# JunweiLiang/FVTA_MemexQA

Measured on AMD Instinct MI355X. Metric: QA-pairs/sec (fwd+bwd) at B=64, 40 photos x 5 streams x 30 tok, h=512, higher is better.
Workload: dtype bf16; 1 GPU; BASELINE.json configs[2] train step (fwd+bwd+adam), shape 'metric', dense lengths; qa_pairs_per_gpu=64, albums=1, photos=40, text_streams=5, hidden=512, global_batch=64, K=6, T=1200, JQ=30, parallelism=dp1 (QA pairs sharded, flat-gradient all-reduce)

## Files before the change

### fvta_memexqa_amd/_lib.py

```python
import ctypes
import os
from ctypes import POINTER, Structure, c_char_p, c_float, c_int, c_int32, c_int64, c_size_t, c_void_p

_HERE = os.path.dirname(os.path.abspath(__file__))
LIB_PATH = os.environ.get("FVTA_LIB_PATH") or os.path.join(_HERE, "csrc", "libfvta_hip.so")

F32, BF16, BF16X3 = 0, 1, 2


class FvtaError(RuntimeError):
    pass


class AttnDesc(Structure):
    _fields_ = [(n, c_int32) for n in ("N", "K", "T", "JQ", "w", "simi", "feat_order", "add_tanh")] + [("hinfo_stride", c_int64)]


class LstmDesc(Structure):
    _fields_ = [(n, c_int32) for n in ("B", "J", "in_", "d", "share_fw_bw", "precision", "training", "reserved", "dx_overwrite", "out_pads_persist")] + \
               [("out_skip", c_int64)]


class TimewarpDesc(Structure):
    _fields_ = [(n, c_int32) for n in ("N", "K", "T", "w", "warp_type")] + [("window_t", c_float)]
# ... 18 lines not shown
class ContextDesc(Structure):
    _fields_ = [(n, c_int32) for n in ("N", "K", "M", "w")] + [("J", c_int32 * CTX_KMAX)]


class GuardDesc(Structure):
    _fields_ = [("grad_scale", c_float), ("clip_value", c_float), ("clip_norm", c_float), ("skip_nonfinite", c_int32),
                ("adam", c_int32), ("lr", c_float), ("beta1", c_float), ("beta2", c_float)]


class GuardCtl(Structure):
    _fields_ = [("grad_scale", c_float), ("clip_value", c_float), ("factor", c_float), ("lr_t", c_float), ("apply", c_int32),
                ("maxabs", c_float), ("norm", ctypes.c_double), ("nonfinite", c_int64), ("applied", c_int64),
                ("skipped", c_int64)]


P = c_void_p
_SIGS = {
    "fvta_version": (c_int, []),
    "fvta_last_error": (c_char_p, []),
    "fvta_abi_struct_bytes": (c_int64, [c_int32]),
    "fvta_attn_workspace_bytes": (c_size_t, [POINTER(AttnDesc)]),
    "fvta_attn_saved_bytes": (c_size_t, [POINTER(AttnDesc)]),
    "fvta_attn_plan": (c_int, [POINTER(AttnDesc), c_int32, POINTER(c_int32)]),
    "fvta_attn_fwd": (c_int, [POINTER(AttnDesc), P, P, P, P, P, P, P, P, P, P, P]),
    "fvta_attn_bwd": (c_int, [POINTER(AttnDesc), P, P, P, P, P, P, P, P, P, P, P, P, c_int, P, P]),
    "fvta_attn_fwd_shadow": (c_int, [POINTER(AttnDesc), P, P, P, P, P, P, P, P, P, P]),
    "fvta_attn_bwd_shadow": (c_int, [POINTER(AttnDesc), P, P, P, P, P, P, P, P, P, P, P, P, c_int, P, P]),
    "fvta_attn_fwd_tw": (c_int, [POINTER(AttnDesc), P, P, P, P, P, P, P, P, P, P, P, P]),
    "fvta_attn_bwd_tw": (c_int, [POINTER(AttnDesc), P, P, P, P, P, P, P, P, P, P, P, P, P, P, c_int, P, P]),
    "fvta_timewarp_bwd_att": (c_int, [POINTER(TimewarpDesc), P, P, P, P, P, P, P, P, P, P, P, P, P, P, P, P, P]),
    "fvta_lstm_plan_bytes": (c_size_t, [POINTER(LstmDesc)]),
    "fvta_lstm_saved_bytes": (c_size_t, [POINTER(LstmDesc)]),
    "fvta_lstm_workspace_bytes": (c_size_t, [POINTER(LstmDesc)]),
    "fvta_lstm_plan": (c_int, [POINTER(LstmDesc), P, P, P, P, c_int64, P, P]),
    "fvta_lstm_plan_xdir": (c_int, [POINTER(LstmDesc), P, P, P, P, c_int64, c_int64, P, P]),
    "fvta_dropout_pair_fwd": (c_int, [P, P, c_int64, c_float, ctypes.c_uint64, P]),
    "fvta_dropout_pair_bwd": (c_int, [P, P, c_int64, c_float, ctypes.c_uint64, c_int32, P]),
    "fvta_bilstm_fwd": (c_int, [POINTER(LstmDesc), P, P, P, P, P, P, P, P, P, P]),
    "fvta_bilstm_bwd": (c_int, [POINTER(LstmDesc), P, P, P, P, P, P, P, P, P, P, P, P, P, P]),
    "fvta_bilstm_bwd_overlap": (c_int, [POINTER(LstmDesc), P, P, P, P, P, P, P, P, P, P, P, P, P, P, P]),
    "fvta_bilstm_bwd_hint": (c_int, [POINTER(LstmDesc), P, P, P, P, P, P, P, P, P, P, P, P, P, P, P, P]),
    "fvta_lstm_shadow_rows": (c_int, [POINTER(LstmDesc), P, P, c_int64, P, P]),
    "fvta_rows_from_shadow": (c_int, [P, c_int64, c_int32, c_int64, P, P]),
    "fvta_lstm_last_state": (c_int, [POINTER(LstmDesc), P, P, c_int32, c_int32, P, P]),
    "fvta_lstm_last_state_bwd": (c_int, [POINTER(LstmDesc), P, P, c_int32, c_int32, P, P]),
    "fvta_scorer_ce_fwd": (c_int, [POINTER(ScorerDesc), P, P, P, P, P, P, P, P, P, P]),
    "fvta_scorer_ce_bwd": (c_int, [POINTER(ScorerDesc), P, P, P, P, P, P, P, P, c_float, P, P, P, P, P, P]),
    "fvta_attgru_fwd": (c_int, [c_int32, c_int32, P, P, P, P, P, P, P, P, P, P]),
    "fvta_attgru_bwd": (c_int, [c_int32, c_int32, P, P, P, P, P, P, P, P, P, P, P, P, P, P, P, P]),
    "fvta_timewarp_workspace_bytes": (c_size_t, [POINTER(TimewarpDesc)]),
    "fvta_timewarp_fwd": (c_int, [POINTER(TimewarpDesc), P, P, P, P, P, P, P, P, P, P, P]),
    "fvta_timewarp_bwd": (c_int, [POINTER(TimewarpDesc), P, P, P, P, P, P, P, P, P, P, P, P, P, P, P, P]),
    "fvta_timewarp_fwd_shadow": (c_int, [POINTER(TimewarpDesc), P, P, P, P, P, P, P, P, P, P, P]),
    "fvta_timewarp_bwd_shadow": (c_int, [POINTER(TimewarpDesc), P, P, P, P, P, P, P, P, P, P, P, P, P, P, P, P]),
    "fvta_embed_workspace_bytes": (c_size_t, [POINTER(EmbedDesc)]),
    "fvta_embed_fwd": (c_int, [POINTER(EmbedDesc), P, P, P, P, P, P, P, P, P, P, P]),
    "fvta_embed_bwd": (c_int, [POINTER(EmbedDesc), P, P, P, P, P, P, P, P, P, P, P, P, P]),
    "fvta_image_trans_fwd": (c_int, [POINTER(ImgTransDesc), P, P, P, P, P, P, P]),
    "fvta_image_trans_bwd": (c_int, [POINTER(ImgTransDesc), P, P, P, P, P, P, P, P, P]),
    "fvta_context_fwd": (c_int, [POINTER(ContextDesc), POINTER(P), POINTER(P), P, P, P]),
    "fvta_context_bwd": (c_int, [POINTER(ContextDesc), P, POINTER(P), P]),
    "fvta_adadelta_step": (c_int, [P, P, P, P, c_int64, c_float, c_float, c_float, c_float, P]),
    "fvta_adam_step": (c_int, [P, P, P, P, c_int64, c_float, c_float, c_float, c_float, c_int32, c_float, P]),
    "fvta_weight_decay": (c_int, [P, P, c_int64, c_float, P, P]),
    "fvta_grad_guard_workspace_bytes": (c_size_t, [c_int64]),
    "fvta_grad_guard": (c_int, [POINTER(GuardDesc), P, c_int64, P, P, P]),
# ... 86 lines not shown
```

### fvta_memexqa_amd/csrc/gemm_bf16.h

```cpp
#pragma once
#include "fvta_common.h"

namespace fvta {

typedef __attribute__((ext_vector_type(8))) __bf16 bf16x8_t;
typedef short s16x4 __attribute__((ext_vector_type(4)));
typedef __attribute__((address_space(3))) void* lds_void_ptr;

union Pack8 {
  bf16x8 s;
  bf16x8_t b;
  f32x4 f;
};

constexpr unsigned GLDS_OOB = 0x80000000u;

__device__ __forceinline__ __amdgpu_buffer_rsrc_t make_rsrc(const void* base, unsigned bytes) {
  return __builtin_amdgcn_make_buffer_rsrc(const_cast<void*>(base), 0, bytes, 0x00020000);
}
__device__ __forceinline__ void glds16(__amdgpu_buffer_rsrc_t rsrc, bf16_t* dst, unsigned voff, unsigned soff) {
  __builtin_amdgcn_raw_ptr_buffer_load_lds(rsrc, (lds_void_ptr)dst, 16, voff, soff, 0, 0);
}
template <int N>
__device__ __forceinline__ void wait_vmcnt() {
// ... 348 lines not shown
  FVTA_LS(2);
  for (int t = 0; t < ntiles; ++t) {
    const int ahead = min(S - 2, ntiles - 1 - t);
    if (ahead >= 3)
      wait_vmcnt<3 * G>();
    else if (ahead == 2)
      wait_vmcnt<2 * G>();
    else if (ahead == 1)
      wait_vmcnt<G>();
    else
      wait_vmcnt<0>();
    FVTA_LS(0);
    __builtin_amdgcn_s_barrier();
    asm volatile("" ::: "memory");
    FVTA_LS(1);
    if (t + S - 1 < ntiles) issue(t + S - 1, a_stage(t + S - 1), a_stage(t + S - 1) + TileCfg::A_ELEMS);
    FVTA_LS(2);
    const bf16_t* As = a_stage(t);
    if constexpr (KMAJOR)
      mma.compute_kmajor(As, As + TileCfg::A_ELEMS);
    else
      mma.compute_rows(As, As + TileCfg::A_ELEMS);
#ifdef FVTA_LOOP_STAMP
    asm volatile("s_nop 0" ::: "memory");
#endif
    FVTA_LS(3);
  }
#ifdef FVTA_LOOP_STAMP
  if (ls_on && mma.lane == 0)
    for (int i = 0; i < 4; ++i) g_loop_stamp[mma.wave_all][i] = ls_sum[i];
#endif
}

}
```

### fvta_memexqa_amd/csrc/lstm.hip

```cpp
#include "gemm_f32.h"
#include "fvta_prof.h"
#include <vector>

#include "lstm_common.h"

namespace fvta {

__device__ const float k_ones4[4] = {1.f, 0.f, 0.f, 0.f};


__global__ __launch_bounds__(1024) void plan_sort_kernel(PlanView v, const int32_t* __restrict__ len_in,
                                                         const int32_t* __restrict__ seq_J_in,
                                                         const int64_t* __restrict__ x_off_in,
                                                         const int64_t* __restrict__ out_off_in,
                                                         int64_t out_ld, int B, int J, int in, int d,
                                                         int64_t x_bw_delta) {
  extern __shared__ int32_t sh[];
  const int tid = threadIdx.x, wave = tid >> 6, lane = tid & 63;
  const int NW = 16, H = J + 1;
  for (int i = tid; i < NW * H; i += 1024) sh[i] = 0;
  const bool fresh = v.hdr->magic != PLAN_MAGIC || v.hdr->B != B || v.hdr->J != J || v.hdr->d != d || v.hdr->out_ld != out_ld;
  __syncthreads();
  if (tid == 0) {
    v.hdr->out_ld = out_ld;
// ... 471 lines not shown
    auto fb = [&](int k, int c, bool& ok) -> const float* { ok = k < K && n0 + c < N; return ok ? B + (size_t)k * N + n0 + c : B; };
    gemm_mainloop(mma, sa, sb, fa, fb, 0, Kp, smem, tid);
  }
#pragma unroll
  for (int ti = 0; ti < 2; ++ti)
#pragma unroll
    for (int r = 0; r < 16; ++r) {
      const int m = m0 + mma.row_of(ti, r);
#pragma unroll
      for (int tj = 0; tj < 2; ++tj) {
        const int n = n0 + mma.col_of(tj);
        if (m < M && n < N) C[(size_t)m * N + n] = mma.acc[ti][tj][r];
      }
    }
}

}

using namespace fvta;

static int check_lstm_desc(const fvta_lstm_desc* d) {
  FVTA_CHECK_ARG(d != nullptr, "lstm: null descriptor");
  FVTA_CHECK_ARG(d->B > 0 && d->J > 0 && d->J <= 1024, "lstm: need B>0 and 0<J<=1024 (B=%d J=%d)", d->B, d->J);
  FVTA_CHECK_ARG(d->in > 0 && d->in % 4 == 0, "lstm: input width must be a positive multiple of 4 (in=%d)", d->in);
  FVTA_CHECK_ARG(d->d > 0 && d->d % 32 == 0, "lstm: hidden size must be a positive multiple of 32 (d=%d)", d->d);
  FVTA_CHECK_ARG(d->precision == FVTA_F32 || d->precision == FVTA_BF16 || d->precision == FVTA_BF16X3,
                 "lstm: unknown precision %d", d->precision);
  return FVTA_OK;
}

extern "C" size_t fvta_lstm_plan_bytes(const fvta_lstm_desc* d) { return plan_view(d, nullptr).bytes; }
extern "C" size_t fvta_lstm_saved_bytes(const fvta_lstm_desc* d) { return saved_view(d, nullptr).bytes; }
extern "C" size_t fvta_lstm_workspace_bytes(const fvta_lstm_desc* d) { return work_view(d, nullptr).bytes; }

extern "C" int fvta_lstm_plan(const fvta_lstm_desc* d, const int32_t* len, const int32_t* seq_J,
                              const int64_t* x_off, const int64_t* out_off, int64_t out_ld, void* plan,
                              fvta_stream_t stream_) {
  return fvta_lstm_plan_xdir(d, len, seq_J, x_off, out_off, out_ld, 0, plan, stream_);
}

extern "C" int fvta_lstm_plan_xdir(const fvta_lstm_desc* d, const int32_t* len, const int32_t* seq_J,
                                   const int64_t* x_off, const int64_t* out_off, int64_t out_ld, int64_t x_bw_delta,
                                   void* plan, fvta_stream_t stream_) {
  if (int e = check_lstm_desc(d)) return e;
  FVTA_CHECK_ARG(len && seq_J && x_off && out_off && plan, "lstm_plan: null pointer");
  FVTA_CHECK_ARG(x_bw_delta >= 0 && x_bw_delta % 4 == 0, "lstm_plan: x_bw_delta=%lld must be >= 0 and a multiple of 4",
                 (long long)x_bw_delta);
  FVTA_CHECK_ARG(out_ld >= 2 * d->d && out_ld % 4 == 0, "lstm_plan: out_ld=%lld must be >= 2d and a multiple of 4",
                 (long long)out_ld);
  hipStream_t stream = (hipStream_t)stream_;
  PlanView v = plan_view(d, plan);
  const size_t sh = (size_t)16 * (d->J + 1) * sizeof(int32_t);
  hipLaunchKernelGGL(plan_sort_kernel, dim3(1), dim3(1024), sh, stream, v, len, seq_J, x_off, out_off, out_ld,
                     d->B, d->J, d->in, d->d, x_bw_delta);
  FVTA_CHECK_LAUNCH("plan_sort");
  hipLaunchKernelGGL(plan_fill_kernel, dim3((d->B + 255) / 256, d->J, 2), dim3(256), 0, stream, v, d->B, d->J,
                     d->in, d->d);
  FVTA_CHECK_LAUNCH("plan_fill");
  return FVTA_OK;
}

extern "C" int fvta_bilstm_fwd(const fvta_lstm_desc* d, const void* plan, const float* x, float* out,
                               const float* kernel_fw, const float* bias_fw, const float* kernel_bw,
                               const float* bias_bw, void* saved, void* workspace, fvta_stream_t stream_) {
  if (int e = check_lstm_desc(d)) return e;
  FVTA_CHECK_ARG(plan && x && out && kernel_fw && bias_fw && workspace, "bilstm_fwd: null pointer");
// ... 117 lines not shown
  s.W[1] = d->share_fw_bw ? kernel_fw : kernel_bw;
  s.dx = dx;
  s.dh_rec = wv.dh_rec;
  s.dzb = wv.dzb;
  s.in_i = in_internal(d);
  const int dbg = fvta_diag_env("FVTA_DEBUG_SKIP", 0);
  s.dbg = dbg;
  s.Wb[0] = wv.wb[0];
  s.Wb[1] = d->share_fw_bw ? wv.wb[0] : wv.wb[1];
  s.B = B;
  s.J = J;
  s.in = in;
  s.d = dd;
  const dim3 ggrid((unsigned)(((size_t)B * dd + 255) / 256), 1, 2);
  const dim3 sgrid((B + MmaSq::BM - 1) / MmaSq::BM, (in + dd + MmaSq::BN - 1) / MmaSq::BN, 2);
  const size_t sh = MmaSq::LDS_FLOATS * sizeof(float);
  DwArgs w;
  w.plan = pv;
  w.x = x;
  w.out = out;
  w.dz = sv.gates;
  w.slabs = wv.slabs;
  w.B = B;
  w.J = J;
  w.in = in;
  w.d = dd;
  w.tgroup = dw_tgroup(d);
  w.nsplit = dw_nsplit(d);
  w.dzb = wv.dzb;
  w.in_i = in_internal(d);
  w.xs = sv.xs;
  w.hs = sv.hs;
  w.xm = lstm_xm(d);
  (void)side_stream_;
  fvta_prof_begin(FVTA_PROF_LSTM_STEP_BWD + 16 * d->reserved, stream);
  if (bf) {
    FusedBwdArgs f;
    f.plan = pv;
    f.Wb[0] = wv.wb[0];
    f.Wb[1] = d->share_fw_bw ? wv.wb[0] : wv.wb[1];
    f.gatesb = sv.gatesb;
    f.cs = sv.cs;
    f.d_out = d_out;
    f.dzb = wv.dzb;
    f.dc = wv.cstate;
    f.dx = dx;
    f.B = B;
    f.J = J;
    f.in = in;
    f.d = dd;
    f.in_i = in_internal(d);
    f.gates32 = sv.gates;
    f.xm = lstm_xm(d);
    f.dx_accumulate = 1;
    f.dx_both = 0;
    if (dx && d->dx_overwrite) {
      const bool direct = dx_writes_whole_rows(f);
      hipLaunchKernelGGL(dx_zero_rows_kernel, dim3((B + 3) / 4), dim3(256), 0, stream, pv, dx, in, direct ? 1 : 0, B);
      f.dx_accumulate = direct ? 0 : 1;
    }
    for (int t = J - 1; t >= 0; --t) {
      f.t = t;
      f.nact_hint = nactive_host ? nactive_host[t] : -1;
      launch_bwd_fused_bf16(f, stream);
    }
    fvta_prof_end(FVTA_PROF_LSTM_STEP_BWD + 16 * d->reserved, J, stream);
    if (dx) {
      fvta_prof_begin(FVTA_PROF_LSTM_DX + 16 * d->reserved, stream);
      launch_dx_bf16(f, stream);
      fvta_prof_end(FVTA_PROF_LSTM_DX + 16 * d->reserved, 1, stream);
    }
  } else {
  if (dx && d->dx_overwrite) hipLaunchKernelGGL(dx_zero_rows_kernel, dim3((B + 3) / 4), dim3(256), 0, stream, pv, dx, in, 0, B);
  for (int t = J - 1; t >= 0; --t) {
    g.t = t;
    s.t = t;
    if (!(dbg & 512)) hipLaunchKernelGGL(lstm_gate_bwd, ggrid, dim3(256), 0, stream, g);
    if (t > 0 || dx) hipLaunchKernelGGL(lstm_step_bwd_f32, sgrid, dim3(256), sh, stream, s);
  }
  }
  if (!bf) fvta_prof_end(FVTA_PROF_LSTM_STEP_BWD + 16 * d->reserved, 2 * J, stream);
  FVTA_CHECK_LAUNCH("lstm_step_bwd");
  const int MM = in + dd + 1, N4 = 4 * dd;
  const dim3 wgrid((MM + MmaSq::BM - 1) / MmaSq::BM, N4 / MmaSq::BN, 2 * w.nsplit);
  fvta_prof_begin(FVTA_PROF_LSTM_DW + 16 * d->reserved, stream);
  if (dbg & 1024) {
  } else if (bf)
    launch_dw_bf16(w, stream);
  else
    hipLaunchKernelGGL(lstm_dw_f32, wgrid, dim3(256), sh, stream, w);
  FVTA_CHECK_LAUNCH("lstm_dw");
  const size_t slab_elems = bf ? (size_t)kpad8(d) * N4 : (size_t)MM * N4;
  const unsigned rgrid = (unsigned)((slab_elems + 255) / 256);
  if (bf) {
    const int ndir = d->share_fw_bw ? 1 : 2;
    for (int i = 0; i < ndir; ++i)
      launch_dw_reduce_bf16(wv.slabs + (size_t)i * w.nsplit * slab_elems, d->share_fw_bw ? 2 * w.nsplit : w.nsplit,
                            in, in_internal(d), dd, i == 0 ? dkernel_fw : dkernel_bw, i == 0 ? dbias_fw : dbias_bw,
                            stream);
  } else if (d->share_fw_bw) {
    hipLaunchKernelGGL(lstm_dw_reduce, dim3(rgrid), dim3(256), 0, stream, wv.slabs, 2 * w.nsplit, slab_elems,
                       in + dd, N4, dkernel_fw, dbias_fw);
  } else {
    hipLaunchKernelGGL(lstm_dw_reduce, dim3(rgrid), dim3(256), 0, stream, wv.slabs, w.nsplit, slab_elems, in + dd,
                       N4, dkernel_fw, dbias_fw);
    hipLaunchKernelGGL(lstm_dw_reduce, dim3(rgrid), dim3(256), 0, stream, wv.slabs + (size_t)w.nsplit * slab_elems,
                       w.nsplit, slab_elems, in + dd, N4, dkernel_bw, dbias_bw);
  }
  fvta_prof_end(FVTA_PROF_LSTM_DW + 16 * d->reserved, 1, stream);
  FVTA_CHECK_LAUNCH("lstm_dw_reduce");
  return FVTA_OK;
}

__global__ __launch_bounds__(256) void shadow_rows_kernel(PlanView v, const bf16_t* __restrict__ hs, int B, int J, int d,
                                                          int64_t nrows, unsigned long long* __restrict__ table) {
  const size_t idx = (size_t)blockIdx.x * blockDim.x + threadIdx.x;
  if (idx >= (size_t)2 * J * B) return;
  const int64_t oo = v.oo[idx];
  if (oo < 0) return;
  const int dir = (int)(idx / ((size_t)J * B));
  const int64_t row = oo / v.hdr->out_ld;
  if (row >= nrows) return;
  table[(size_t)dir * nrows + row] = (unsigned long long)reinterpret_cast<uintptr_t>(hs + idx * (size_t)d);
}
extern "C" int fvta_lstm_shadow_rows(const fvta_lstm_desc* d, const void* plan, const void* saved, int64_t nrows,
                                     uint64_t* table, fvta_stream_t stream) {
  if (int e = check_lstm_desc(d)) return e;
  FVTA_CHECK_ARG(plan && saved && table && nrows > 0, "lstm_shadow_rows: null pointer / no rows");
  FVTA_CHECK_ARG(d->precision == FVTA_BF16, "lstm_shadow_rows: the bf16 engine's shadow rows only");
  PlanView pv = plan_view(d, const_cast<void*>(plan));
// ... 79 lines not shown
```

### fvta_memexqa_amd/csrc/lstm_bf16.hip

```cpp
#include "gemm_bf16.h"
#include <type_traits>
#include "lstm_common.h"

namespace fvta {

static inline int pad8(int v) { return (v + 7) / 8 * 8; }

template <int B, int E, class F>
__device__ __forceinline__ void bf_static_for(F&& f) {
  if constexpr (B < E) {
    f(std::integral_constant<int, B>{});
    bf_static_for<B + 1, E>(f);
  }
}

template <class K>
static void allow_big_lds(K kernel, int bytes) {
  (void)hipFuncSetAttribute(reinterpret_cast<const void*>(kernel), hipFuncAttributeMaxDynamicSharedMemorySize, bytes);
}

__device__ __forceinline__ int il32(int e) { return ((e >> 5) << 6) + (e & 31); }
__global__ void cvt_weights_kernel(const float* __restrict__ W, bf16_t* __restrict__ wt, bf16_t* __restrict__ wb,
                                   int in, int in_i, int d, int xm) {
  __shared__ float tile[32][33];
// ... 557 lines not shown
    }
    for (int dir = 0; dir < 2; ++dir)
      hipLaunchKernelGGL((lstm_dx_bf16<2, FVTA_DX_BK, FVTA_DX_ST, false, false, XM>), grid, dim3(512), LDS, s, a, dir, a.dx_accumulate || dir);
    return;
  }
  constexpr int NBK = XM == 1 ? 32 : 64, NST = XM == 1 ? 3 : 2;
  if (XM == 2 && a.B <= 64 && a.in <= 128) {
    constexpr int LDSP = TileCfgT<4, 2, 1, NST, NBK, 1>::LDS_BYTES + 64 * 8;
    allow_big_lds(lstm_dx_bf16<4, NBK, NST, false, false, XM, 1, 1>, LDSP);
    const dim3 gridp((a.B + 63) / 64, 1, a.J);
    for (int dir = 0; dir < 2; ++dir)
      hipLaunchKernelGGL((lstm_dx_bf16<4, NBK, NST, false, false, XM, 1, 1>), gridp, dim3(256), LDSP, s, a, dir, a.dx_accumulate || dir);
    return;
  }
  constexpr int LDS1 = TileCfgT<1, 2, 4, NST, NBK>::LDS_BYTES + 256 * 8;
  allow_big_lds(lstm_dx_bf16<1, NBK, NST, false, false, XM>, LDS1);
  const dim3 grid(pad8((a.B + 255) / 256), (a.in + 127) / 128, a.J);
  for (int dir = 0; dir < 2; ++dir)
    hipLaunchKernelGGL((lstm_dx_bf16<1, NBK, NST, false, false, XM>), grid, dim3(256), LDS1, s, a, dir, a.dx_accumulate || dir);
}

void launch_dx_bf16(const FusedBwdArgs& a, hipStream_t s) {
  if (a.xm == 2)
    launch_dx_xm<2>(a, s);
  else
    launch_dx_xm<1>(a, s);
}

#ifndef FVTA_DW_STAGES
#define FVTA_DW_STAGES 4
#endif
constexpr int dw_stages(int wn) { return wn == 2 ? FVTA_DW_STAGES : 3; }

template <int WN>
__global__ __launch_bounds__((TileCfgT<WN>::NT), (WN == 1 ? 2 : 1)) void lstm_dw_bf16(DwArgs a) {
  typedef TileCfgT<WN, 2, 4, dw_stages(WN)> TileCfg;
  typedef MmaBT<WN, 2, 4, dw_stages(WN)> MmaB;
  extern __shared__ __attribute__((aligned(16))) bf16_t smem_h[];
  const int tid = threadIdx.x;
  const int d = a.d, in_i = a.in_i, N4 = 4 * d;
  const int xtiles = (in_i + TileCfg::BM - 1) / TileCfg::BM;
  const int mtiles = xtiles + (d + TileCfg::BM - 1) / TileCfg::BM, ntiles = N4 / TileCfg::BN, per = mtiles * ntiles;
  const int xcd = blockIdx.x & 7, slot = blockIdx.x >> 3;
  const int bz = xcd + 8 * (slot / per);
  const int tile_id = slot % per;
  if (bz >= 2 * a.nsplit) return;
  const int bx = tile_id % mtiles, by = tile_id / mtiles;
  const bool isx = bx < xtiles;
  const int col0 = isx ? bx * TileCfg::BM : (bx - xtiles) * TileCfg::BM;
  const int ncols = isx ? in_i : d;
  const int n0 = by * TileCfg::BN;
  const int split = bz % a.nsplit, dir = bz / a.nsplit;
  MmaB mma;
  mma.init(tid);
  KMajorSrc<TileCfg::BM, TileCfg::A_GLDS> sa;
  KMajorSrc<TileCfg::BN, TileCfg::B_GLDS> sb;
  sa.setup(mma.wave_all, mma.lane, col0, ncols, (unsigned)ncols * 2);
  sb.setup(mma.wave_all, mma.lane, n0, N4, (unsigned)N4 * 2);
  const int t_begin = split * a.tgroup, t_end = min(a.J, t_begin + a.tgroup);
  for (int t = t_begin; t < t_end; ++t) {
    const int nact = a.plan.nactive[t];
    if (nact == 0) break;
    if (!isx && t == 0) continue;
    const size_t trow = ((size_t)dir * a.J + t) * a.B;
    const bf16_t* A = isx ? a.xs + trow * in_i : a.hs + (trow - (size_t)a.B) * d;
    const __amdgpu_buffer_rsrc_t ra = make_rsrc(A, (unsigned)nact * ncols * 2);
    const __amdgpu_buffer_rsrc_t rz = make_rsrc(a.dzb + trow * (size_t)N4, (unsigned)nact * N4 * 2);
    auto issue = [&](int tile, bf16_t* As, bf16_t* Bs) {
      sa.issue(ra, As, mma.wave_all, (unsigned)tile * 32u * ncols * 2u);
      sb.issue(rz, Bs, mma.wave_all, (unsigned)tile * 32u * N4 * 2u);
    };
    glds_mainloop<true>(mma, issue, (nact + 31) / 32, smem_h);
    __builtin_amdgcn_s_barrier();
  }
  float* slab = a.slabs + (size_t)bz * (in_i + d) * N4;
  const int mrow0 = isx ? col0 : in_i + col0;
#pragma unroll
  for (int ti = 0; ti < MmaB::TM; ++ti)
#pragma unroll
    for (int r = 0; r < 16; ++r) {
      const int ml = mma.row_of(ti, r);
      if (col0 + ml >= ncols) continue;
#pragma unroll
      for (int tj = 0; tj < MmaB::TN; ++tj) slab[(size_t)(mrow0 + ml) * N4 + n0 + mma.col_of(tj)] = mma.acc[ti][tj][r];
    }
}

__global__ __launch_bounds__(512, 1) void lstm_dw_x2(DwArgs a) {
  typedef DwX2Cfg TileCfg;
  extern __shared__ __attribute__((aligned(16))) bf16_t smem_h[];
  const int tid = threadIdx.x;
  const int d = a.d, in_i = a.in_i, N4 = 4 * d;
  const int xtiles = (in_i + TileCfg::BM - 1) / TileCfg::BM;
  const int mtiles = xtiles + (d + TileCfg::BM - 1) / TileCfg::BM, ntiles = (N4 + TileCfg::BN - 1) / TileCfg::BN, per = mtiles * ntiles;
  const int xcd = blockIdx.x & 7, slot = blockIdx.x >> 3;
  const int bz = xcd + 8 * (slot / per);
  const int tile_id = slot % per;
  if (bz >= 2 * a.nsplit) return;
  const int bx = tile_id % mtiles, by = tile_id / mtiles;
  const bool isx = bx < xtiles;
  const int col0 = isx ? bx * TileCfg::BM : (bx - xtiles) * TileCfg::BM;
  const int ncols = isx ? in_i : d;
  const int n0 = by * TileCfg::BN;
  const int split = bz % a.nsplit, dir = bz / a.nsplit;
  MmaX2K mma;
  mma.init(tid);
  KMajorSrc<TileCfg::PCOLS, TileCfg::A_GLDS> sa;
  KMajorSrc<TileCfg::PCOLS, TileCfg::B_GLDS> sb;
  sa.setup(mma.wave_all, mma.lane, 2 * col0, 2 * ncols, (unsigned)ncols * 4);
  sb.setup(mma.wave_all, mma.lane, 2 * n0, 2 * N4, (unsigned)N4 * 4);
  const int t_begin = split * a.tgroup, t_end = min(a.J, t_begin + a.tgroup);
  for (int t = t_begin; t < t_end; ++t) {
    const int nact = a.plan.nactive[t];
    if (nact == 0) break;
    if (!isx && t == 0) continue;
    const size_t trow = ((size_t)dir * a.J + t) * a.B;
    const bf16_t* A = isx ? a.xs + trow * (size_t)(2 * in_i) : a.hs + (trow - (size_t)a.B) * (size_t)(2 * d);
    const __amdgpu_buffer_rsrc_t ra = make_rsrc(A, (unsigned)nact * ncols * 4);
    const __amdgpu_buffer_rsrc_t rz = make_rsrc(a.dzb + trow * (size_t)(2 * N4), (unsigned)nact * N4 * 4);
    auto issue = [&](int tile, bf16_t* As, bf16_t* Bs) {
      sa.issue(ra, As, mma.wave_all, (unsigned)tile * TileCfg::KR * ncols * 4u);
      sb.issue(rz, Bs, mma.wave_all, (unsigned)tile * TileCfg::KR * N4 * 4u);
    };
    glds_mainloop<true>(mma, issue, (nact + TileCfg::KR - 1) / TileCfg::KR, smem_h);
    __builtin_amdgcn_s_barrier();
  }
  float* slab = a.slabs + (size_t)bz * (in_i + d) * N4;
  const int mrow0 = isx ? col0 : in_i + col0;
#pragma unroll
  for (int ti = 0; ti < MmaX2K::TM; ++ti)
#pragma unroll
    for (int r = 0; r < 16; ++r) {
      const int ml = mma.row_of(ti, r);
      if (col0 + ml >= ncols) continue;
#pragma unroll
      for (int tj = 0; tj < MmaX2K::TN; ++tj)
        if (n0 + mma.col_of(tj) < N4) slab[(size_t)(mrow0 + ml) * N4 + n0 + mma.col_of(tj)] = mma.acc[ti][tj][r];
    }
}

void launch_dw_bf16(const DwArgs& a, hipStream_t s) {
  const int slices8 = (2 * a.nsplit + 7) / 8;
  if (a.xm == 2) {
    allow_big_lds(lstm_dw_x2, DwX2Cfg::LDS_BYTES);
    const int per = ((a.in_i + 255) / 256 + (a.d + 255) / 256) * ((4 * a.d + 255) / 256);
    hipLaunchKernelGGL(lstm_dw_x2, dim3(8 * per * slices8), dim3(512), DwX2Cfg::LDS_BYTES, s, a);
    return;
  }
  if ((4 * a.d) % 256 == 0) {
    constexpr int LDS2 = TileCfgT<2, 2, 4, dw_stages(2)>::LDS_BYTES;
    allow_big_lds(lstm_dw_bf16<2>, LDS2);
    const int per = ((a.in_i + 255) / 256 + (a.d + 255) / 256) * (4 * a.d / 256);
    hipLaunchKernelGGL((lstm_dw_bf16<2>), dim3(8 * per * slices8), dim3(512), LDS2, s, a);
  } else {
    allow_big_lds(lstm_dw_bf16<1>, TileCfgT<1>::LDS_BYTES);
    const int per = ((a.in_i + 255) / 256 + (a.d + 255) / 256) * (4 * a.d / 128);
    hipLaunchKernelGGL((lstm_dw_bf16<1>), dim3(8 * per * slices8), dim3(256), TileCfgT<1>::LDS_BYTES, s, a);
  }
}

__global__ __launch_bounds__(256) void lstm_dw_reduce_bf16(const float* __restrict__ slabs, int nslab, int in, int in_i, int d,
                                                            float* __restrict__ dW, float* __restrict__ dbias) {
  const int N4 = 4 * d;
  const size_t slab_elems = (size_t)(in_i + d) * N4;
  const size_t idx = ((size_t)blockIdx.x * blockDim.x + threadIdx.x) * 4;
  if (idx >= slab_elems) return;
  const int row = (int)(idx / N4), u = (int)(idx % N4) >> 2;
  if (row > in && row < in_i) return;
  f32x4 s = f32x4{0.f, 0.f, 0.f, 0.f};
  int k = 0;
  for (; k + 8 <= nslab; k += 8) {
    f32x4 v[8];
#pragma unroll
    for (int j = 0; j < 8; ++j) v[j] = *reinterpret_cast<const f32x4*>(slabs + (size_t)(k + j) * slab_elems + idx);
#pragma unroll
// ... 184 lines not shown
```

### fvta_memexqa_amd/csrc/lstm_common.h

```cpp
#pragma once
#include "fvta_common.h"

namespace fvta {

struct PlanHeader {
  int64_t out_ld;
  int32_t B, J, in, d;
  int64_t x_bw_delta;
  uint32_t magic;
  int32_t pad[7];
};
constexpr uint32_t PLAN_MAGIC = 0x46565441u;

struct PlanView {
  PlanHeader* hdr;
  int32_t* order;
  int32_t* nactive;
  int32_t* len;
  int32_t* seq_J;
  int64_t* x_off;
  int64_t* out_off;
  int64_t* xo;
  int64_t* oo;
  int32_t* dirty;
// ... 29 lines not shown
  bf16_t* gatesb;
  float* cs;
  bf16_t* xs;
  bf16_t* hs;
  size_t bytes;
};
static inline SavedView saved_view(const fvta_lstm_desc* d, void* p) {
  FvtaCarver c(p);
  SavedView s;
  s.gates = s.cs = nullptr;
  s.xs = s.hs = s.gatesb = nullptr;
  if (d->training) {
    if (d->precision == FVTA_BF16)
      s.gatesb = c.take<bf16_t>((size_t)2 * d->J * d->B * 4 * d->d);
    else
      s.gates = c.take<float>((size_t)2 * d->J * d->B * 4 * d->d);
    s.cs = c.take<float>((size_t)2 * d->J * d->B * d->d);
  }
  if (lstm_is_bf(d)) {
    s.xs = c.take<bf16_t>((size_t)2 * d->J * d->B * in_internal(d) * lstm_xm(d));
    s.hs = c.take<bf16_t>((size_t)2 * d->J * d->B * d->d * lstm_xm(d));
  }
  s.bytes = c.off < 256 ? 256 : c.off;
  return s;
}

static inline int dw_tgroup(const fvta_lstm_desc* d) {
  int g = (d->J + 15) / 16;
  return g < 1 ? 1 : g;
}
static inline int dw_nsplit(const fvta_lstm_desc* d) { return (d->J + dw_tgroup(d) - 1) / dw_tgroup(d); }
static inline int kpad8(const fvta_lstm_desc* d) { return in_internal(d) + d->d; }

struct WorkView {
  float* cstate;
  float* dh_rec;
  float* slabs;
  bf16_t* wt[2];
  bf16_t* wb[2];
  bf16_t* dzb;
  bf16_t* wf[2];
  size_t bytes;
};
static inline WorkView work_view(const fvta_lstm_desc* d, void* p) {
  FvtaCarver c(p);
  WorkView w;
  w.cstate = c.take<float>((size_t)2 * d->B * d->d);
  w.dh_rec = c.take<float>((size_t)2 * d->B * d->d);
  const size_t slab_rows = lstm_is_bf(d) ? (size_t)kpad8(d) : (size_t)(d->in + d->d + 1);
  w.slabs = c.take<float>((size_t)2 * dw_nsplit(d) * slab_rows * 4 * d->d);
  w.wt[0] = w.wt[1] = w.wb[0] = w.wb[1] = nullptr;
  w.dzb = nullptr;
  w.wf[0] = w.wf[1] = nullptr;
  if (lstm_is_bf(d)) {
    const size_t xm = (size_t)lstm_xm(d);
    for (int i = 0; i < 2; ++i) {
      w.wt[i] = c.take<bf16_t>((size_t)4 * d->d * kpad8(d) * xm);
      w.wb[i] = c.take<bf16_t>((size_t)kpad8(d) * 4 * d->d * xm);
    }
    if (d->training) w.dzb = c.take<bf16_t>((size_t)2 * d->J * d->B * 4 * d->d * xm);
    for (int i = 0; i < 2; ++i) w.wf[i] = c.take<bf16_t>((size_t)4 * d->d * kpad8(d) * xm);
  }
  w.bytes = c.off;
  return w;
}

struct StepArgs {
  PlanView plan;
  const float* x;
  float* out;
  const float* W[2];
  const bf16_t* Wt[2];
  const bf16_t* Wf[2];
  const bf16_t* xs;
  bf16_t* hs;
  const float* bias[2];
  float* gates;
  bf16_t* gatesb;
  float* cs;
  float* cstate;
  int t, B, J, in, d, Kp;
  int dbg;
  int xm;
  int nt;
  int64_t out_skip;
};

struct GateBwdArgs {
  PlanView plan;
  const float* d_out;
  float* gates;
  const bf16_t* gatesb;
  bf16_t* dzb;
  const float* cs;
  float* dc;
  float* dh_rec;
  int t, B, J, d;
};

struct StepBwdArgs {
  PlanView plan;
  const float* dz;
  const bf16_t* dzb;
  const float* W[2];
  const bf16_t* Wb[2];
  float* dx;
  float* dh_rec;
  int t, B, J, in, d, in_i;
  int dbg;
};

struct DwArgs {
  PlanView plan;
  const float* x;
  const float* out;
  const float* dz;
  const bf16_t* dzb;
  const bf16_t* xs;
  const bf16_t* hs;
  float* slabs;
  int B, J, in, d, tgroup, nsplit, in_i;
  int xm;
};

#ifdef __HIPCC__
template <class Mma>
__device__ __forceinline__ void lstm_gate_epilogue(const Mma& mma, const StepArgs& a, int dir, int m0, int u0,
                                                   int nact, size_t trow, const int64_t* s_oo) {
  static_assert(Mma::TN == 4 && Mma::WAVES_N == 1, "wave tile must span the four gate strips");
  const int d = a.d, t = a.t;
  const float* __restrict__ bias = a.bias[dir];
  const int u = u0 + mma.l31;
  const float bi = bias[u], bj = bias[d + u], bf = bias[2 * d + u], bo = bias[3 * d + u];
  const float* cprev_src = a.cs ? a.cs + (trow - a.B) * (size_t)d : a.cstate + (size_t)dir * a.B * d;
#pragma unroll
  for (int ti = 0; ti < Mma::TM; ++ti) {
    float cp[16];
#pragma unroll
    for (int r = 0; r < 16; ++r) {
      const int i = min(m0 + mma.row_of(ti, r), nact - 1);
      cp[r] = (t > 0 && !(a.dbg & 64)) ? cprev_src[(size_t)i * d + u] : 0.f;
    }
#pragma unroll
    for (int r = 0; r < 16; ++r) {
      const int row = mma.row_of(ti, r);
      const int i = m0 + row;
      const float ig = fvta_sigmoid(mma.acc[ti][0][r] + bi);
      const float jg = fvta_tanh(mma.acc[ti][1][r] + bj);
      const float fg = fvta_sigmoid(mma.acc[ti][2][r] + bf + 1.0f);
      const float og = fvta_sigmoid(mma.acc[ti][3][r] + bo);
      const float c = cp[r] * fg + ig * jg;
      const float h = fvta_tanh(c) * og;
      if (i < nact) {
        if (a.cs) {
          if (!(a.dbg & 16)) a.cs[(trow + i) * d + u] = c;
// ... 194 lines not shown
```

### include/fvta_hip.h

```cpp
#ifndef FVTA_HIP_H
#define FVTA_HIP_H

#include <stddef.h>
#include <stdint.h>

#ifdef __cplusplus
extern "C" {
#endif

#define FVTA_OK 0
#define FVTA_ERR_INVALID_ARG (-1)
#define FVTA_ERR_LAUNCH (-2)
#define FVTA_ERR_UNSUPPORTED (-3)

#define FVTA_F32 0
#define FVTA_BF16 1
#define FVTA_BF16X3 2

typedef void* fvta_stream_t;

int fvta_version(void);
const char* fvta_last_error(void);
int64_t fvta_abi_struct_bytes(int32_t which);

// ... 21 lines not shown
int fvta_attn_fwd_shadow(const fvta_attn_desc* d, const uint64_t* table, const float* hq, const uint8_t* hmask,
                         const uint8_t* qmask, const float* W, const float* b, float* h_a, void* saved, void* workspace,
                         fvta_stream_t stream);
int fvta_attn_bwd_shadow(const fvta_attn_desc* d, const uint64_t* table, const float* hq, const uint8_t* hmask,
                         const uint8_t* qmask, const float* W, const float* b, const float* d_h_a, const void* saved,
                         float* d_hinfo, float* d_hq, float* dW, float* db, int accumulate, void* workspace,
                         fvta_stream_t stream);

int fvta_attn_fwd_tw(const fvta_attn_desc* d, const float* hinfo, const float* hq, const uint8_t* hmask,
                     const uint8_t* qmask, const float* W, const float* b, const float* tscale, float* h_a,
                     float* a_logits, void* saved, void* workspace, fvta_stream_t stream);
int fvta_attn_bwd_tw(const fvta_attn_desc* d, const float* hinfo, const float* hq, const uint8_t* hmask,
                     const uint8_t* qmask, const float* W, const float* b, const float* tscale, const float* d_h_a,
                     const void* saved, float* d_hinfo, float* d_hq, float* dW, float* db, float* d_tscale,
                     int accumulate, void* workspace, fvta_stream_t stream);

typedef struct fvta_lstm_desc {
  int32_t B;
  int32_t J;
  int32_t in;
  int32_t d;
  int32_t share_fw_bw;
  int32_t precision;
  int32_t training;
  int32_t reserved;
  int32_t dx_overwrite;
  int32_t out_pads_persist;
  int64_t out_skip;
} fvta_lstm_desc;

size_t fvta_lstm_plan_bytes(const fvta_lstm_desc* d);
size_t fvta_lstm_saved_bytes(const fvta_lstm_desc* d);
size_t fvta_lstm_workspace_bytes(const fvta_lstm_desc* d);

int fvta_lstm_plan(const fvta_lstm_desc* d, const int32_t* len, const int32_t* seq_J, const int64_t* x_off,
                   const int64_t* out_off, int64_t out_ld, void* plan, fvta_stream_t stream);

int fvta_lstm_plan_xdir(const fvta_lstm_desc* d, const int32_t* len, const int32_t* seq_J, const int64_t* x_off,
                        const int64_t* out_off, int64_t out_ld, int64_t x_bw_delta, void* plan, fvta_stream_t stream);
int fvta_dropout_pair_fwd(const float* x, float* x2, int64_t n, float keep_prob, uint64_t seed, fvta_stream_t stream);
int fvta_dropout_pair_bwd(const float* dx2, float* dx, int64_t n, float keep_prob, uint64_t seed, int32_t accumulate,
                          fvta_stream_t stream);

int fvta_bilstm_fwd(const fvta_lstm_desc* d, const void* plan, const float* x, float* out,
                    const float* kernel_fw, const float* bias_fw, const float* kernel_bw,
                    const float* bias_bw, void* saved, void* workspace, fvta_stream_t stream);

int fvta_bilstm_bwd(const fvta_lstm_desc* d, const void* plan, const float* x, const float* out,
                    const float* d_out, const float* kernel_fw, const float* kernel_bw, void* saved,
                    float* dx, float* dkernel_fw, float* dbias_fw, float* dkernel_bw, float* dbias_bw,
                    void* workspace, fvta_stream_t stream);

int fvta_bilstm_bwd_overlap(const fvta_lstm_desc* d, const void* plan, const float* x, const float* out,
                            const float* d_out, const float* kernel_fw, const float* kernel_bw, void* saved,
                            float* dx, float* dkernel_fw, float* dbias_fw, float* dkernel_bw, float* dbias_bw,
                            void* workspace, fvta_stream_t stream, fvta_stream_t side_stream);

int fvta_bilstm_bwd_hint(const fvta_lstm_desc* d, const void* plan, const float* x, const float* out,
                         const float* d_out, const float* kernel_fw, const float* kernel_bw, void* saved,
                         float* dx, float* dkernel_fw, float* dbias_fw, float* dkernel_bw, float* dbias_bw,
                         void* workspace, fvta_stream_t stream, fvta_stream_t side_stream, const int32_t* nactive_host);

int fvta_lstm_shadow_rows(const fvta_lstm_desc* d, const void* plan, const void* saved, int64_t nrows, uint64_t* table,
                          fvta_stream_t stream);
int fvta_rows_from_shadow(const uint64_t* table, int64_t nrows, int32_t d, int64_t out_ld, float* out, fvta_stream_t stream);
int fvta_lstm_last_state(const fvta_lstm_desc* d, const void* plan, const float* out, int32_t s0,
// ... 202 lines not shown
```

Measured before the change: 5402 QA-pairs/s.

## Balance LSTM weight-gradient work by k-tile slices across timesteps

```diff
diff --git a/fvta_memexqa_amd/_lib.py b/fvta_memexqa_amd/_lib.py
--- a/fvta_memexqa_amd/_lib.py
+++ b/fvta_memexqa_amd/_lib.py
@@ -74,6 +74,8 @@
     "fvta_lstm_plan_bytes": (c_size_t, [POINTER(LstmDesc)]),
     "fvta_lstm_saved_bytes": (c_size_t, [POINTER(LstmDesc)]),
     "fvta_lstm_workspace_bytes": (c_size_t, [POINTER(LstmDesc)]),
+    "fvta_lstm_dw_nslices": (c_int, [POINTER(LstmDesc)]),
+    "fvta_lstm_dw_slices": (c_int, [POINTER(c_int32), c_int32, c_int32, c_int32, c_int32, POINTER(c_int32)]),
     "fvta_lstm_plan": (c_int, [POINTER(LstmDesc), P, P, P, P, c_int64, P, P]),
     "fvta_lstm_plan_xdir": (c_int, [POINTER(LstmDesc), P, P, P, P, c_int64, c_int64, P, P]),
     "fvta_dropout_pair_fwd": (c_int, [P, P, c_int64, c_float, ctypes.c_uint64, P]),
diff --git a/fvta_memexqa_amd/csrc/gemm_bf16.h b/fvta_memexqa_amd/csrc/gemm_bf16.h
--- a/fvta_memexqa_amd/csrc/gemm_bf16.h
+++ b/fvta_memexqa_amd/csrc/gemm_bf16.h
@@ -404,4 +404,38 @@
 #endif
 }
 
-}
+template <class Mma, class Cursor>
+__device__ __forceinline__ void glds_mainloop_kmajor_steps(Mma& mma, Cursor& cur, int ntiles, bf16_t* smem) {
+  typedef typename Mma::Cfg TileCfg;
+  constexpr int S = TileCfg::STAGES, G = TileCfg::A_GLDS + TileCfg::B_GLDS;
+  static_assert(S >= 3 && S <= 5, "ring depth");
+  if (ntiles <= 0) return;
+#pragma unroll
+  for (int p = 0; p < S - 1; ++p) {
+    bf16_t* st = smem + p * TileCfg::STAGE_ELEMS;
+    cur.issue(st, st + TileCfg::A_ELEMS);
+    cur.advance();
+    cur.prefetch();
+    cur.settle();
+  }
+  cur.prefetch();
+  int is = S - 1, cs = 0;
+  for (int i = 0; i < ntiles; ++i) {
+    wait_vmcnt<(S - 2) * G>();
+    __builtin_amdgcn_s_barrier();
+    asm volatile("" ::: "memory");
+    cur.settle();
+    bf16_t* st = smem + is * TileCfg::STAGE_ELEMS;
+    cur.issue(st, st + TileCfg::A_ELEMS);
+    cur.advance();
+    const bf16_t* As = smem + cs * TileCfg::STAGE_ELEMS;
+    mma.compute_kmajor(As, As + TileCfg::A_ELEMS);
+    cur.prefetch();
+    is = is + 1 == S ? 0 : is + 1;
+    cs = cs + 1 == S ? 0 : cs + 1;
+  }
+  cur.settle();
+  wait_vmcnt<0>();
+}
+
+}
diff --git a/fvta_memexqa_amd/csrc/lstm.hip b/fvta_memexqa_amd/csrc/lstm.hip
--- a/fvta_memexqa_amd/csrc/lstm.hip
+++ b/fvta_memexqa_amd/csrc/lstm.hip
@@ -527,6 +527,30 @@
 extern "C" size_t fvta_lstm_plan_bytes(const fvta_lstm_desc* d) { return plan_view(d, nullptr).bytes; }
 extern "C" size_t fvta_lstm_saved_bytes(const fvta_lstm_desc* d) { return saved_view(d, nullptr).bytes; }
 extern "C" size_t fvta_lstm_workspace_bytes(const fvta_lstm_desc* d) { return work_view(d, nullptr).bytes; }
+
+extern "C" int fvta_lstm_dw_nslices(const fvta_lstm_desc* d) {
+  if (check_lstm_desc(d)) return -1;
+  return lstm_is_bf(d) ? dw_nslices(d) : 0;
+}
+extern "C" int fvta_lstm_dw_slices(const int32_t* nactive, int32_t J, int32_t KR, int32_t NS, int32_t htile, int32_t* out) {
+  FVTA_CHECK_ARG(nactive && out, "lstm_dw_slices: null pointer");
+  FVTA_CHECK_ARG(J > 0 && KR > 0 && NS > 0, "lstm_dw_slices: need J, KR, NS > 0 (J=%d KR=%d NS=%d)", J, KR, NS);
+  for (int t = 0; t < J; ++t)
+    FVTA_CHECK_ARG(nactive[t] >= 0 && (t == 0 || nactive[t] <= nactive[t - 1]),
+                   "lstm_dw_slices: nactive must be non-negative and non-increasing (step %d)", t);
+  for (int s = 0; s < NS; ++s) {
+    const DwSlice sl = dw_slice_range(nactive, J, KR, NS, s, htile != 0);
+    int32_t* o = out + 5 * s;
+    o[0] = o[1] = o[2] = o[3] = -1;
+    o[4] = sl.n;
+    if (sl.n <= 0) continue;
+    int t = sl.t, k = sl.k;
+    for (int i = 1; i < sl.n; ++i)
+      if (++k >= dw_ktiles(nactive[t], KR)) ++t, k = 0;
+    o[0] = sl.t, o[1] = sl.k, o[2] = t, o[3] = k;
+  }
+  return FVTA_OK;
+}
 
 extern "C" int fvta_lstm_plan(const fvta_lstm_desc* d, const int32_t* len, const int32_t* seq_J,
                               const int64_t* x_off, const int64_t* out_off, int64_t out_ld, void* plan,
@@ -710,6 +734,7 @@
   w.xs = sv.xs;
   w.hs = sv.hs;
   w.xm = lstm_xm(d);
+  w.nslices = bf ? dw_nslices(d) : 0;
   (void)side_stream_;
   fvta_prof_begin(FVTA_PROF_LSTM_STEP_BWD + 16 * d->reserved, stream);
   if (bf) {
@@ -773,7 +798,7 @@
   if (bf) {
     const int ndir = d->share_fw_bw ? 1 : 2;
     for (int i = 0; i < ndir; ++i)
-      launch_dw_reduce_bf16(wv.slabs + (size_t)i * w.nsplit * slab_elems, d->share_fw_bw ? 2 * w.nsplit : w.nsplit,
+      launch_dw_reduce_bf16(wv.slabs + (size_t)i * w.nslices * slab_elems, d->share_fw_bw ? 2 * w.nslices : w.nslices,
                             in, in_internal(d), dd, i == 0 ? dkernel_fw : dkernel_bw, i == 0 ? dbias_fw : dbias_bw,
                             stream);
   } else if (d->share_fw_bw) {
diff --git a/fvta_memexqa_amd/csrc/lstm_bf16.hip b/fvta_memexqa_amd/csrc/lstm_bf16.hip
--- a/fvta_memexqa_amd/csrc/lstm_bf16.hip
+++ b/fvta_memexqa_amd/csrc/lstm_bf16.hip
@@ -613,6 +613,71 @@
 #endif
 constexpr int dw_stages(int wn) { return wn == 2 ? FVTA_DW_STAGES : 3; }
 
+
+struct DwPlace {
+  int bz;
+  int dir, slice, col0, ncols, n0;
+  bool isx;
+};
+template <int BM, int BN>
+__device__ __forceinline__ DwPlace dw_place(const DwArgs& a) {
+  const int N4 = 4 * a.d;
+  const int xtiles = (a.in_i + BM - 1) / BM;
+  const int mtiles = xtiles + (a.d + BM - 1) / BM, ntiles = (N4 + BN - 1) / BN, per = mtiles * ntiles;
+  const int xcd = blockIdx.x & 7, slot = blockIdx.x >> 3;
+  const int tile_id = slot % per, bx = tile_id % mtiles, by = tile_id / mtiles;
+  DwPlace p;
+  p.bz = xcd + 8 * (slot / per);
+  p.isx = bx < xtiles;
+  p.col0 = p.isx ? bx * BM : (bx - xtiles) * BM;
+  p.ncols = p.isx ? a.in_i : a.d;
+  p.n0 = by * BN;
+  p.slice = p.bz % a.nslices, p.dir = p.bz / a.nslices;
+  return p;
+}
+
+typedef const __attribute__((address_space(4))) int32_t* dw_nact_ptr;
+template <int KR, class SA, class SB>
+struct DwCursor {
+  const SA& sa;
+  const SB& sb;
+  dw_nact_ptr nactive;
+  const bf16_t *abase, *zbase;
+  int a_back;
+  size_t a_step, z_step;
+  unsigned a_ld, z_ld;
+  int J, wave;
+  int t, k, nk, nact, nact_nx, left;
+  __device__ __forceinline__ DwCursor(const SA& sa_, const SB& sb_) : sa(sa_), sb(sb_) {}
+  __device__ __forceinline__ void start(const DwSlice& sl) {
+    t = sl.t, k = sl.k, left = sl.n;
+    nact = nactive[min(t, J)];
+    nk = dw_ktiles(nact, KR);
+    prefetch();
+    settle();
+  }
+  __device__ __forceinline__ void issue(bf16_t* As, bf16_t* Bs) const {
+    const unsigned rows = left > 0 ? (unsigned)nact : 0u;
+    const __amdgpu_buffer_rsrc_t ra = make_rsrc(abase + (size_t)(t - a_back) * a_step, rows * a_ld);
+    const __amdgpu_buffer_rsrc_t rz = make_rsrc(zbase + (size_t)t * z_step, rows * z_ld);
+    sa.issue(ra, As, wave, (unsigned)k * KR * a_ld);
+    sb.issue(rz, Bs, wave, (unsigned)k * KR * z_ld);
+  }
+  __device__ __forceinline__ void advance() {
+    const bool wrap = k + 1 >= nk;
+    left -= 1;
+    k = wrap ? 0 : k + 1;
+    t = wrap ? t + 1 : t;
+    nact = wrap ? nact_nx : nact;
+    nk = dw_ktiles(nact, KR);
+  }
+  __device__ __forceinline__ void prefetch() {
+    dw_nact_ptr p = nactive + min(t + 1, J);
+    asm volatile("s_load_dword %0, %1, 0x0" : "=s"(nact_nx) : "s"(p) : "memory");
+  }
+  __device__ __forceinline__ void settle() { asm volatile("s_waitcnt lgkmcnt(0)" : "+s"(nact_nx)::"memory"); }
+};
+
 template <int WN>
 __global__ __launch_bounds__((TileCfgT<WN>::NT), (WN == 1 ? 2 : 1)) void lstm_dw_bf16(DwArgs a) {
   typedef TileCfgT<WN, 2, 4, dw_stages(WN)> TileCfg;
@@ -620,41 +685,31 @@
   extern __shared__ __attribute__((aligned(16))) bf16_t smem_h[];
   const int tid = threadIdx.x;
   const int d = a.d, in_i = a.in_i, N4 = 4 * d;
-  const int xtiles = (in_i + TileCfg::BM - 1) / TileCfg::BM;
-  const int mtiles = xtiles + (d + TileCfg::BM - 1) / TileCfg::BM, ntiles = N4 / TileCfg::BN, per = mtiles * ntiles;
-  const int xcd = blockIdx.x & 7, slot = blockIdx.x >> 3;
-  const int bz = xcd + 8 * (slot / per);
-  const int tile_id = slot % per;
-  if (bz >= 2 * a.nsplit) return;
-  const int bx = tile_id % mtiles, by = tile_id / mtiles;
-  const bool isx = bx < xtiles;
-  const int col0 = isx ? bx * TileCfg::BM : (bx - xtiles) * TileCfg::BM;
-  const int ncols = isx ? in_i : d;
-  const int n0 = by * TileCfg::BN;
-  const int split = bz % a.nsplit, dir = bz / a.nsplit;
+  const DwPlace p = dw_place<TileCfg::BM, TileCfg::BN>(a);
+  if (p.bz >= 2 * a.nslices) return;
+  const bool isx = p.isx;
+  const int col0 = p.col0, ncols = p.ncols, n0 = p.n0;
   MmaB mma;
   mma.init(tid);
-  KMajorSrc<TileCfg::BM, TileCfg::A_GLDS> sa;
-  KMajorSrc<TileCfg::BN, TileCfg::B_GLDS> sb;
+  typedef KMajorSrc<TileCfg::BM, TileCfg::A_GLDS> SrcA;
+  typedef KMajorSrc<TileCfg::BN, TileCfg::B_GLDS> SrcB;
+  SrcA sa;
+  SrcB sb;
   sa.setup(mma.wave_all, mma.lane, col0, ncols, (unsigned)ncols * 2);
   sb.setup(mma.wave_all, mma.lane, n0, N4, (unsigned)N4 * 2);
-  const int t_begin = split * a.tgroup, t_end = min(a.J, t_begin + a.tgroup);
-  for (int t = t_begin; t < t_end; ++t) {
-    const int nact = a.plan.nactive[t];
-    if (nact == 0) break;
-    if (!isx && t == 0) continue;
-    const size_t trow = ((size_t)dir * a.J + t) * a.B;
-    const bf16_t* A = isx ? a.xs + trow * in_i : a.hs + (trow - (size_t)a.B) * d;
-    const __amdgpu_buffer_rsrc_t ra = make_rsrc(A, (unsigned)nact * ncols * 2);
-    const __amdgpu_buffer_rsrc_t rz = make_rsrc(a.dzb + trow * (size_t)N4, (unsigned)nact * N4 * 2);
-    auto issue = [&](int tile, bf16_t* As, bf16_t* Bs) {
-      sa.issue(ra, As, mma.wave_all, (unsigned)tile * 32u * ncols * 2u);
-      sb.issue(rz, Bs, mma.wave_all, (unsigned)tile * 32u * N4 * 2u);
-    };
-    glds_mainloop<true>(mma, issue, (nact + 31) / 32, smem_h);
-    __builtin_amdgcn_s_barrier();
-  }
-  float* slab = a.slabs + (size_t)bz * (in_i + d) * N4;
+  DwCursor<32, SrcA, SrcB> cur(sa, sb);
+  cur.nactive = (dw_nact_ptr)a.plan.nactive;
+  cur.J = a.J, cur.wave = mma.wave_all;
+  const size_t row0 = (size_t)p.dir * a.J * a.B;
+  cur.abase = isx ? a.xs + row0 * in_i : a.hs + row0 * d;
+  cur.a_back = isx ? 0 : 1;
+  cur.zbase = a.dzb + row0 * (size_t)N4;
+  cur.a_step = (size_t)a.B * ncols, cur.z_step = (size_t)a.B * N4;
+  cur.a_ld = (unsigned)ncols * 2, cur.z_ld = (unsigned)N4 * 2;
+  const DwSlice sl = dw_slice_range(cur.nactive, a.J, 32, a.nslices, p.slice, !isx);
+  cur.start(sl);
+  glds_mainloop_kmajor_steps(mma, cur, sl.n, smem_h);
+  float* slab = a.slabs + (size_t)p.bz * (in_i + d) * N4;
   const int mrow0 = isx ? col0 : in_i + col0;
 #pragma unroll
   for (int ti = 0; ti < MmaB::TM; ++ti)
@@ -672,41 +727,31 @@
   extern __shared__ __attribute__((aligned(16))) bf16_t smem_h[];
   const int tid = threadIdx.x;
   const int d = a.d, in_i = a.in_i, N4 = 4 * d;
-  const int xtiles = (in_i + TileCfg::BM - 1) / TileCfg::BM;
-  const int mtiles = xtiles + (d + TileCfg::BM - 1) / TileCfg::BM, ntiles = (N4 + TileCfg::BN - 1) / TileCfg::BN, per = mtiles * ntiles;
-  const int xcd = blockIdx.x & 7, slot = blockIdx.x >> 3;
-  const int bz = xcd + 8 * (slot / per);
-  const int tile_id = slot % per;
-  if (bz >= 2 * a.nsplit) return;
-  const int bx = tile_id % mtiles, by = tile_id / mtiles;
-  const bool isx = bx < xtiles;
-  const int col0 = isx ? bx * TileCfg::BM : (bx - xtiles) * TileCfg::BM;
-  const int ncols = isx ? in_i : d;
-  const int n0 = by * TileCfg::BN;
-  const int split = bz % a.nsplit, dir = bz / a.nsplit;
+  const DwPlace p = dw_place<TileCfg::BM, TileCfg::BN>(a);
+  if (p.bz >= 2 * a.nslices) return;
+  const bool isx = p.isx;
+  const int col0 = p.col0, ncols = p.ncols, n0 = p.n0;
   MmaX2K mma;
   mma.init(tid);
-  KMajorSrc<TileCfg::PCOLS, TileCfg::A_GLDS> sa;
-  KMajorSrc<TileCfg::PCOLS, TileCfg::B_GLDS> sb;
+  typedef KMajorSrc<TileCfg::PCOLS, TileCfg::A_GLDS> SrcA;
+  typedef KMajorSrc<TileCfg::PCOLS, TileCfg::B_GLDS> SrcB;
+  SrcA sa;
+  SrcB sb;
   sa.setup(mma.wave_all, mma.lane, 2 * col0, 2 * ncols, (unsigned)ncols * 4);
   sb.setup(mma.wave_all, mma.lane, 2 * n0, 2 * N4, (unsigned)N4 * 4);
-  const int t_begin = split * a.tgroup, t_end = min(a.J, t_begin + a.tgroup);
-  for (int t = t_begin; t < t_end; ++t) {
-    const int nact = a.plan.nactive[t];
-    if (nact == 0) break;
-    if (!isx && t == 0) continue;
-    const size_t trow = ((size_t)dir * a.J + t) * a.B;
-    const bf16_t* A = isx ? a.xs + trow * (size_t)(2 * in_i) : a.hs + (trow - (size_t)a.B) * (size_t)(2 * d);
-    const __amdgpu_buffer_rsrc_t ra = make_rsrc(A, (unsigned)nact * ncols * 4);
-    const __amdgpu_buffer_rsrc_t rz = make_rsrc(a.dzb + trow * (size_t)(2 * N4), (unsigned)nact * N4 * 4);
-    auto issue = [&](int tile, bf16_t* As, bf16_t* Bs) {
-      sa.issue(ra, As, mma.wave_all, (unsigned)tile * TileCfg::KR * ncols * 4u);
-      sb.issue(rz, Bs, mma.wave_all, (unsigned)tile * TileCfg::KR * N4 * 4u);
-    };
-    glds_mainloop<true>(mma, issue, (nact + TileCfg::KR - 1) / TileCfg::KR, smem_h);
-    __builtin_amdgcn_s_barrier();
-  }
-  float* slab = a.slabs + (size_t)bz * (in_i + d) * N4;
+  DwCursor<TileCfg::KR, SrcA, SrcB> cur(sa, sb);
+  cur.nactive = (dw_nact_ptr)a.plan.nactive;
+  cur.J = a.J, cur.wave = mma.wave_all;
+  const size_t row0 = (size_t)p.dir * a.J * a.B;
+  cur.abase = isx ? a.xs + row0 * (size_t)(2 * in_i) : a.hs + row0 * (size_t)(2 * d);
+  cur.a_back = isx ? 0 : 1;
+  cur.zbase = a.dzb + row0 * (size_t)(2 * N4);
+  cur.a_step = (size_t)a.B * 2 * ncols, cur.z_step = (size_t)a.B * 2 * N4;
+  cur.a_ld = (unsigned)ncols * 4, cur.z_ld = (unsigned)N4 * 4;
+  const DwSlice sl = dw_slice_range(cur.nactive, a.J, TileCfg::KR, a.nslices, p.slice, !isx);
+  cur.start(sl);
+  glds_mainloop_kmajor_steps(mma, cur, sl.n, smem_h);
+  float* slab = a.slabs + (size_t)p.bz * (in_i + d) * N4;
   const int mrow0 = isx ? col0 : in_i + col0;
 #pragma unroll
   for (int ti = 0; ti < MmaX2K::TM; ++ti)
@@ -721,7 +766,7 @@
 }
 
 void launch_dw_bf16(const DwArgs& a, hipStream_t s) {
-  const int slices8 = (2 * a.nsplit + 7) / 8;
+  const int slices8 = (2 * a.nslices + 7) / 8;
   if (a.xm == 2) {
     allow_big_lds(lstm_dw_x2, DwX2Cfg::LDS_BYTES);
     const int per = ((a.in_i + 255) / 256 + (a.d + 255) / 256) * ((4 * a.d + 255) / 256);
diff --git a/fvta_memexqa_amd/csrc/lstm_common.h b/fvta_memexqa_amd/csrc/lstm_common.h
--- a/fvta_memexqa_amd/csrc/lstm_common.h
+++ b/fvta_memexqa_amd/csrc/lstm_common.h
@@ -85,6 +85,64 @@
 static inline int dw_nsplit(const fvta_lstm_desc* d) { return (d->J + dw_tgroup(d) - 1) / dw_tgroup(d); }
 static inline int kpad8(const fvta_lstm_desc* d) { return in_internal(d) + d->d; }
 
+#if defined(__HIPCC__)
+#define FVTA_HD __host__ __device__
+#else
+#define FVTA_HD
+#endif
+struct DwSlice {
+  int t, k;
+  int n;
+};
+FVTA_HD inline int dw_ktiles(int nact, int KR) { return nact > 0 ? (nact + KR - 1) / KR : 0; }
+template <class NactPtr>
+FVTA_HD inline DwSlice dw_slice_range(NactPtr nactive, int J, int KR, int NS, int s, bool htile) {
+  const int tb = htile ? 1 : 0;
+  long long T = 0;
+  for (int t0 = tb; t0 < J; t0 += 8) {
+    int nk[8];
+#pragma unroll
+    for (int u = 0; u < 8; ++u) nk[u] = dw_ktiles(nactive[t0 + u < J ? t0 + u : J - 1], KR);
+#pragma unroll
+    for (int u = 0; u < 8; ++u) T += t0 + u < J ? nk[u] : 0;
+  }
+  const long long lo = s * T / NS, hi = (s + 1) * T / NS;
+  DwSlice r;
+  r.t = tb;
+  r.k = 0;
+  r.n = (int)(hi - lo);
+  long long before = 0;
+  bool found = false;
+  for (int t0 = tb; t0 < J && !found; t0 += 8) {
+    int nk[8];
+#pragma unroll
+    for (int u = 0; u < 8; ++u) nk[u] = dw_ktiles(nactive[t0 + u < J ? t0 + u : J - 1], KR);
+#pragma unroll
+    for (int u = 0; u < 8; ++u) {
+      const bool here = !found && t0 + u < J && lo < before + nk[u];
+      r.t = here ? t0 + u : r.t;
+      r.k = here ? (int)(lo - before) : r.k;
+      found = found || here;
+      before += nk[u];
+    }
+  }
+  return r;
+}
+#ifndef FVTA_DW_SLICE_KTILES
+#define FVTA_DW_SLICE_KTILES 32
+#endif
+static inline int dw_kr(const fvta_lstm_desc* d) { return d->precision == FVTA_BF16X3 ? 16 : 32; }
+static inline int dw_nslices(const fvta_lstm_desc* d) {
+  const long long kmax = (long long)d->J * ((d->B + dw_kr(d) - 1) / dw_kr(d));
+  for (int ns = 16; ns > 4; ns -= 4)
+    if (kmax >= (long long)FVTA_DW_SLICE_KTILES * ns) return ns;
+  return 4;
+}
+static inline int dw_nslabs(const fvta_lstm_desc* d) {
+  const int a = dw_nsplit(d), b = lstm_is_bf(d) ? dw_nslices(d) : 0;
+  return a > b ? a : b;
+}
+
 struct WorkView {
   float* cstate;
   float* dh_rec;
@@ -101,7 +159,6 @@
   w.cstate = c.take<float>((size_t)2 * d->B * d->d);
   w.dh_rec = c.take<float>((size_t)2 * d->B * d->d);
   const size_t slab_rows = lstm_is_bf(d) ? (size_t)kpad8(d) : (size_t)(d->in + d->d + 1);
-  w.slabs = c.take<float>((size_t)2 * dw_nsplit(d) * slab_rows * 4 * d->d);
   w.wt[0] = w.wt[1] = w.wb[0] = w.wb[1] = nullptr;
   w.dzb = nullptr;
   w.wf[0] = w.wf[1] = nullptr;
@@ -114,6 +171,7 @@
     if (d->training) w.dzb = c.take<bf16_t>((size_t)2 * d->J * d->B * 4 * d->d * xm);
     for (int i = 0; i < 2; ++i) w.wf[i] = c.take<bf16_t>((size_t)4 * d->d * kpad8(d) * xm);
   }
+  w.slabs = c.take<float>((size_t)2 * dw_nslabs(d) * slab_rows * 4 * d->d);
   w.bytes = c.off;
   return w;
 }
@@ -174,6 +232,7 @@
   float* slabs;
   int B, J, in, d, tgroup, nsplit, in_i;
   int xm;
+  int nslices;
 };
 
 #ifdef __HIPCC__
diff --git a/include/fvta_hip.h b/include/fvta_hip.h
--- a/include/fvta_hip.h
+++ b/include/fvta_hip.h
@@ -77,6 +77,9 @@
 size_t fvta_lstm_plan_bytes(const fvta_lstm_desc* d);
 size_t fvta_lstm_saved_bytes(const fvta_lstm_desc* d);
 size_t fvta_lstm_workspace_bytes(const fvta_lstm_desc* d);
+
+int fvta_lstm_dw_nslices(const fvta_lstm_desc* d);
+int fvta_lstm_dw_slices(const int32_t* nactive, int32_t J, int32_t KR, int32_t NS, int32_t htile, int32_t* out);
 
 int fvta_lstm_plan(const fvta_lstm_desc* d, const int32_t* len, const int32_t* seq_J, const int64_t* x_off,
                    const int64_t* out_off, int64_t out_ld, void* plan, fvta_stream_t stream);
```

After: 5330 QA-pairs/s. 1.3% lower.
